# AnonymWriter/Iris-Style-Transfer

Measured on NVIDIA B200. Metric: masked-NST image-steps/sec @640x400 VGG-19, higher is better.
Workload: dtype bf16

## Files before the change

### include/isx.h

```cpp
#ifndef ISX_H_
#define ISX_H_

#include <stdint.h>

#ifdef __cplusplus
extern "C" {
#endif

#define ISX_VERSION 100

typedef uint16_t isx_bf16;
typedef void* isx_stream;

const char* isx_last_error(void);
int isx_version(void);
int isx_device_check(int device);

int isx_ipc_export(const void* ptr, void* handle64, int64_t* offset);
int isx_ipc_open(const void* handle64, void** base_out);
int isx_ipc_close(void* base);
int isx_copy_d2d_async(void* dst, const void* src, int64_t bytes, isx_stream stream);

typedef void* isx_handle;
int isx_create(int device, isx_handle* out);
// ... 20 lines not shown
                              int H, int W, int Cin, int Cout, int relu, int tile_cfg, isx_stream stream);

int isx_conv3x3_bias_relu_pool_fwd(const isx_bf16* in, const isx_bf16* w_fwd, const float* bias, isx_bf16* out,
                                   isx_bf16* pool_out, int B, int H, int W, int Cin, int Cout, int tile_cfg,
                                   isx_stream stream);
int isx_conv3x3_bias_relu_pool_idx_fwd(const isx_bf16* in, const isx_bf16* w_fwd, const float* bias, isx_bf16* out,
                                       isx_bf16* pool_out, uint8_t* pool_idx, int skip_out, int B, int H, int W, int Cin,
                                       int Cout, int tile_cfg, isx_stream stream);

int isx_conv3x3_dgrad(const isx_bf16* dy, const isx_bf16* w_dgrad, isx_bf16* dx, int B, int H, int W, int Cin,
                      int Cout, const isx_bf16* relu_act, const isx_bf16* add_grad, const float* aff_a,
                      const float* aff_b, int tile_cfg, isx_stream stream);

int isx_conv3x3_dgrad_gram(const isx_bf16* dy, const isx_bf16* w_dgrad, isx_bf16* dx, int B, int H, int W, int Cin,
                           int Cout, const isx_bf16* act_below, const isx_bf16* gram_D, isx_stream stream);

int isx_maxpool2x2_fwd(const isx_bf16* in, isx_bf16* out, int B, int H, int W, int C, isx_stream stream);
int isx_maxpool2x2_bwd(const isx_bf16* dy_pooled, const isx_bf16* act_prepool, isx_bf16* dx, int B, int H, int W,
                       int C, isx_stream stream);
int isx_maxpool2x2_fwd_idx(const isx_bf16* in, isx_bf16* out, uint8_t* idx, int B, int H, int W, int C, isx_stream stream);
int isx_maxpool2x2_bwd_idx(const isx_bf16* dy_pooled, const uint8_t* idx, isx_bf16* dx, int B, int H, int W, int C,
                           isx_stream stream);

int64_t isx_gram_workspace_bytes(int B, int HW, int C);
int isx_gram_fwd(const isx_bf16* feat, int B, int HW, int C, float inv_n, void* workspace, float* G_out,
                 const float* target, int target_b, double loss_scale, double* loss, float grad_scale,
                 isx_bf16* D_out, isx_stream stream);
int64_t isx_gram_mask_flags_bytes(int mask_b, int HW, int C);
int isx_gram_masked_fwd(const isx_bf16* feat, int B, int HW, int C, const float* m, int mask_b, void* flags_ws,
                        isx_bf16* fm2, float inv_n, void* workspace, float* G_out, const float* target, int target_b,
// ... 144 lines not shown
```

### iris-style-transfer_b200/csrc/api_ops.cu

```cuda
#include "../../include/isx.h"
#include "isx_common.cuh"
#include "isx_internal.h"
#include "isx_kernels.h"

using namespace isx;
typedef __nv_bfloat16 bf16;

static inline cudaStream_t S(isx_stream s) { return reinterpret_cast<cudaStream_t>(s); }
static inline const bf16* P(const isx_bf16* p) { return reinterpret_cast<const bf16*>(p); }
static inline bf16* P(isx_bf16* p) { return reinterpret_cast<bf16*>(p); }

static void decode_tile_cfg(int cfg, ConvArgs* a) {
  if (cfg > 0) {
    a->force_bn = cfg / 100;
    a->force_mt = (cfg % 100) / 10;
    a->force_stages = cfg % 10;
  }
}

extern "C" int isx_pack_conv3x3_weights(const float* w, int Cout, int Cin, isx_bf16* wf, isx_bf16* wd,
                                        isx_stream stream) {
  ISX_REQUIRE(w && (wf || wd) && Cout > 0 && Cin > 0, "isx_pack_conv3x3_weights: bad arguments");
  return pack_conv_weights(w, Cout, Cin, P(wf), P(wd), S(stream));
}
// ... 84 lines not shown
  a.in = P(dy); a.weight = P(w_dgrad); a.out = P(dx);
  a.B = B; a.H = H; a.W = W; a.Cin = Cout; a.Cout = Cin; a.ntaps = 9;
  a.mask_act = P(relu_act); a.add_buf = P(add_grad); a.aff_a = aff_a; a.aff_b = aff_b;
  decode_tile_cfg(tile_cfg, &a);
  return conv_tc(a, S(stream));
}

extern "C" int isx_conv3x3_dgrad_gram(const isx_bf16* dy, const isx_bf16* w_dgrad, isx_bf16* dx, int B, int H, int W,
                                      int Cin, int Cout, const isx_bf16* act_below, const isx_bf16* gram_D,
                                      isx_stream stream) {
  ISX_REQUIRE(dy && w_dgrad && dx && act_below && gram_D, "isx_conv3x3_dgrad_gram: null pointer");
  ConvArgs a;
  a.in = P(dy); a.weight = P(w_dgrad); a.out = P(dx);
  a.B = B; a.H = H; a.W = W; a.Cin = Cout; a.Cout = Cin; a.ntaps = 9;
  a.mask_act = P(act_below); a.gram_act = P(act_below); a.gram_D = P(gram_D);
  return conv_tc(a, S(stream));
}

extern "C" int isx_maxpool2x2_fwd(const isx_bf16* in, isx_bf16* out, int B, int H, int W, int C, isx_stream stream) {
  ISX_REQUIRE(in && out, "isx_maxpool2x2_fwd: null pointer");
  return maxpool_fwd(P(in), P(out), B, H, W, C, S(stream));
}

extern "C" int isx_maxpool2x2_bwd(const isx_bf16* dy, const isx_bf16* act, isx_bf16* dx, int B, int H, int W, int C,
                                  isx_stream stream) {
  ISX_REQUIRE(dy && act && dx, "isx_maxpool2x2_bwd: null pointer");
  return maxpool_bwd(P(dy), P(act), P(dx), B, H, W, C, S(stream));
}

extern "C" int isx_maxpool2x2_fwd_idx(const isx_bf16* in, isx_bf16* out, uint8_t* idx, int B, int H, int W, int C,
// ... 159 lines not shown
```

### iris-style-transfer_b200/csrc/conv_c64.cu

```cuda
#include <algorithm>

#include "isx_common.cuh"
#include "isx_internal.h"
#include "isx_kernels.h"

namespace isx {

static constexpr int kC64Threads = 64 + 256;
static constexpr int kHalo = 18 * 16 * 128;
static constexpr int kTile = 128 * 128;

struct C64Params {
  int B, H, W, Cout;
  int tiles_x, tiles_y;
  long total_items;
  int halo_slots;
  int relu, fuse_pool, use_mask, use_gram;
  const float* bias;
  const __nv_bfloat16* add_buf;
  const float* aff_a;
  const float* aff_b;
  float* dx_nchw;
  int xc;
  const float* in_mask;
// ... 387 lines not shown
      if (isx_make_tmap_bf16(&tmP, a.pool_out, 4, dp, sp, bp, true)) return 3;
    }
  }
  auto kern = conv_c64_kernel<BN, EPI>;
  ISX_CHECK_CUDA(cudaFuncSetAttribute(kern, cudaFuncAttributeMaxDynamicSharedMemorySize, (int)smem_bytes));
  const long grid = std::min<long>(p.total_items, kNumSMs);
  isx_prof_begin(ISX_PROF_CONV, 2.0 * (9 * 64 + (p.use_gram ? a.Cout : 0)) * a.Cout * static_cast<double>(a.B) * a.H * a.W, stream);
  kern<<<(unsigned)grid, kC64Threads, smem_bytes, stream>>>(tmA, tmW, tmO, tmM, tmD, tmP, p);
  isx_prof_end(ISX_PROF_CONV, stream);
  ISX_LAUNCH_CHECK();
  return 0;
}

bool conv_c64_applicable(const ConvArgs& a) {
  if (a.Cin != 64 || a.ntaps != 9 || a.per_image_weights) return false;
  if (a.dx_nchw != nullptr) return a.Cout == 16;
  if (a.Cout != 64) return false;
  if (a.gram_act != nullptr && a.gram_act != a.mask_act) return false;
  return true;
}

int conv_c64(const ConvArgs& a, cudaStream_t stream) {
  ISX_REQUIRE(conv_c64_applicable(a), "conv_c64: not applicable");
  if (a.dx_nchw != nullptr) return launch_c64<16, 1>(a, stream);
  return launch_c64<64, 0>(a, stream);
}

}
```

### iris-style-transfer_b200/csrc/conv_halo.cu

```cuda
#include <algorithm>

#include "isx_common.cuh"
#include "isx_internal.h"
#include "isx_kernels.h"

namespace isx {

static constexpr int kHaloThreads = 64 + 256;
static constexpr int kHaloSlot = 43 * 1024;
static constexpr int kSub = 128 * 128;

struct HaloParams {
  int B, H, W, Cin, Cout;
  int pairs_x, pairs_y, n_tiles;
  int total_items;
  int cin_blocks, extra_kb;
  int w_stages;
  int relu, fuse_pool, use_mask;
  const float* bias;
  const __nv_bfloat16* add_buf;
  const float* aff_a;
  const float* aff_b;
  uint8_t* pool_idx;
  int skip_out;
};

struct HaloLayout {
  int halo, w, act, stg, pstg, bars, total;
};
template <int BN>
__host__ __device__ inline HaloLayout halo_layout(int w_stages, int use_mask, int fuse_pool) {
  HaloLayout L;
  int off = 0;
  L.halo = off; off += 2 * kHaloSlot;
  L.w = off; off += w_stages * BN * 128;
  L.act = off; off += use_mask ? 2 * kSub : 0;
  L.stg = off; off += 2 * kSub;
  L.pstg = off; off += fuse_pool ? 2 * 4096 : 0;
  L.bars = off; off += 512;
  L.total = off;
  return L;
}

template <bool VERT>
struct ItemWalk {
  int b, r, stride, per_img, pairs_x, n_tiles;
  __device__ ItemWalk(int first, int stride_, int per_img_, int pairs_x_, int n_tiles_)
      : b(first / per_img_), r(first % per_img_), stride(stride_), per_img(per_img_), pairs_x(pairs_x_), n_tiles(n_tiles_) {}
  __device__ void next() {
    r += stride;
    while (r >= per_img) { r -= per_img; ++b; }
  }
  __device__ int nt() const { return r % n_tiles; }
// ... 6 lines not shown
conv_halo_kernel(const __grid_constant__ CUtensorMap tmA, const __grid_constant__ CUtensorMap tmW,
                 const __grid_constant__ CUtensorMap tmO, const __grid_constant__ CUtensorMap tmM,
                 const __grid_constant__ CUtensorMap tmA2, const __grid_constant__ CUtensorMap tmD,
                 const __grid_constant__ CUtensorMap tmP, const HaloParams p) {
  constexpr int kPitch = VERT ? 10 : 18;
  constexpr int kPatchRows = VERT ? 34 : 18;
  constexpr int kHaloBytes = kPitch * kPatchRows * 128;
  constexpr int kMtOff = VERT ? 16 * kPitch * 128 : 8 * 128;
  constexpr int kWStage = BN * 128;
  constexpr int kNH = BN / 64;
  constexpr int kNSub = 2 * kNH;
  constexpr int kAccCols = 2 * BN;
  constexpr int kTmemCols = 2 * kAccCols;
  extern __shared__ uint8_t smem_raw[];
  uint8_t* smem = reinterpret_cast<uint8_t*>((reinterpret_cast<uintptr_t>(smem_raw) + 1023) & ~uintptr_t(1023));
  const HaloLayout L = halo_layout<BN>(p.w_stages, p.use_mask, p.fuse_pool);
  const int WS = p.w_stages;
  uint64_t* bars = reinterpret_cast<uint64_t*>(smem + L.bars);
  uint64_t* halo_full = bars;
  uint64_t* halo_empty = bars + 2;
  uint64_t* w_full = bars + 4;
  uint64_t* w_empty = bars + 12;
  uint64_t* act_full = bars + 20;
  uint64_t* tmem_full = bars + 22;
  uint64_t* tmem_empty = bars + 24;
  uint32_t* tmem_ptr_smem = reinterpret_cast<uint32_t*>(bars + 26);

  const int warp = threadIdx.x >> 5;
  const int lane = threadIdx.x & 31;

  if (warp == 0 && lane == 0) {
// ... 138 lines not shown
    const int tw = row & 7, th = row >> 3;
    const bool leader = threadIdx.x == 64;
    ItemWalk<VERT> it(blockIdx.x, gridDim.x, per_img, p.pairs_x, p.n_tiles);
    auto issue_mask_load = [&](const ItemWalk<VERT>& w, int s, uint32_t g) {
      const int mt = s / kNH, nh = s - mt * kNH;
      const uint32_t slot = g & 1;
      mbar_arrive_expect_tx(&act_full[slot], kSub);
      tma_load_4d(smem + L.act + slot * kSub, &tmM, &act_full[slot], w.nt() * BN + nh * 64,
                  w.x0() + (VERT ? 0 : 8 * mt), w.y0() + (VERT ? 16 * mt : 0), w.b);
    };
    uint32_t g = 0;
    if (p.use_mask && leader && n_my > 0) {
      issue_mask_load(it, 0, 0);
      issue_mask_load(it, 1, 1);
    }
    uint32_t acc = 0, aph = 0;
    for (int i = 0; i < n_my; ++i) {
      const int b = it.b, x0 = it.x0(), y0 = it.y0(), n0 = it.nt() * BN;
      ItemWalk<VERT> nxt = it;
      nxt.next();
      mbar_wait(&tmem_full[acc], aph);
      tc_fence_after();
#pragma unroll 1
      for (int s = 0; s < kNSub; ++s, ++g) {
        const int mt = s / kNH, nh = s - mt * kNH;
        const int xs = x0 + (VERT ? 0 : 8 * mt), ys = y0 + (VERT ? 16 * mt : 0);
        const int nc = n0 + nh * 64 + hsel * 32;
        const int x = xs + tw, y = ys + th;
        const bool valid = (x < p.W) && (y < p.H);
        const size_t pix = valid ? ((static_cast<size_t>(b) * p.H + y) * p.W + x) * p.Cout : 0;
// ... 59 lines not shown
#pragma unroll
        for (int c = 0; c < 4; ++c) {
          uint4 o;
          o.x = pack_bf16x2(f[c * 8 + 0], f[c * 8 + 1]);
          o.y = pack_bf16x2(f[c * 8 + 2], f[c * 8 + 3]);
          o.z = pack_bf16x2(f[c * 8 + 4], f[c * 8 + 5]);
          o.w = pack_bf16x2(f[c * 8 + 6], f[c * 8 + 7]);
          const int chunk = (hsel * 4 + c) ^ (row & 7);
          *reinterpret_cast<uint4*>(rowp + chunk * 16) = o;
        }
        fence_proxy_async_smem();
        if (leader) tma_store_wait_read<0>();
        asm volatile("bar.sync 1, 256;" ::: "memory");
        const bool inside = xs < p.W && ys < p.H;
        if (leader) {
          if (inside && !p.skip_out) {
            tma_store_4d(&tmO, stg, n0 + nh * 64, xs, ys, b);
            tma_store_commit();
          }
          if (p.use_mask) {
            if (s + 2 < kNSub) issue_mask_load(it, s + 2, g + 2);
            else if (i + 1 < n_my) issue_mask_load(nxt, s + 2 - kNSub, g + 2);
          }
        }
        if (p.fuse_pool) {
          uint8_t* pst = smem + L.pstg + slot * 4096;
          const int item = threadIdx.x - 64;
          const int pr = item >> 3, chunk = item & 7;
          const int px = pr & 3, py = pr >> 2;
          const int r00 = (2 * py) * 8 + 2 * px;
          const int rr[4] = {r00, r00 + 1, r00 + 8, r00 + 9};
          uint4 u4[4];
#pragma unroll
          for (int k = 0; k < 4; ++k) u4[k] = *reinterpret_cast<const uint4*>(stg + rr[k] * 128 + ((chunk ^ (rr[k] & 7)) * 16));
          uint4 m4;
          uint2 codes;
          pool4_codes(u4, m4, codes);
          if (p.pool_idx != nullptr) {
// ... 32 lines not shown
  memset(&p, 0, sizeof(p));
  p.B = a.B; p.H = a.H; p.W = a.W; p.Cin = a.Cin; p.Cout = a.Cout;
  p.pairs_x = VERT ? (a.W + 7) / 8 : (a.W + 15) / 16;
  p.pairs_y = VERT ? (a.H + 31) / 32 : (a.H + 15) / 16;
  p.n_tiles = a.Cout / BN;
  const long total = static_cast<long>(p.pairs_x) * p.pairs_y * p.n_tiles * a.B;
  ISX_REQUIRE(total < (1L << 31) - kNumSMs, "conv_halo: too many work items");
  p.total_items = static_cast<int>(total);
  p.cin_blocks = a.Cin / 64;
  p.extra_kb = a.gram_act != nullptr ? a.Cout / 64 : 0;
  p.relu = a.relu; p.bias = a.bias; p.add_buf = a.add_buf; p.aff_a = a.aff_a; p.aff_b = a.aff_b;
  p.use_mask = a.mask_act != nullptr ? 1 : 0;
  p.fuse_pool = (a.pool_out != nullptr && a.H >= 2 && a.W >= 2) ? 1 : 0;
  p.pool_idx = p.fuse_pool ? a.pool_idx : nullptr;
  p.skip_out = (p.fuse_pool && a.pool_idx != nullptr && a.skip_out) ? 1 : 0;
  int ws = 6;
  HaloLayout L = halo_layout<BN>(ws, p.use_mask, p.fuse_pool);
  const int cap = (227 - std::max(0, std::min(isx_ctx()->opt_smem_reserve_kb, 22))) * 1024;
  while (ws > 2 && 1024 + L.total > cap) { --ws; L = halo_layout<BN>(ws, p.use_mask, p.fuse_pool); }
  ISX_REQUIRE(1024 + L.total <= 227 * 1024, "conv_halo: %d B of shared memory exceed 227 KB", 1024 + L.total);
  p.w_stages = ws;
  const size_t smem_bytes = std::max<size_t>(1024 + L.total, 204 * 1024);

  CUtensorMap tmA, tmW, tmO, tmM, tmA2, tmD, tmP;
  {
    uint64_t dims[4] = {(uint64_t)a.Cin, (uint64_t)a.W, (uint64_t)a.H, (uint64_t)a.B};
    uint64_t str[3] = {(uint64_t)a.Cin * 2, (uint64_t)a.W * a.Cin * 2, (uint64_t)a.H * a.W * a.Cin * 2};
    uint32_t box[4] = {64, VERT ? 10u : 18u, VERT ? 34u : 18u, 1};
    if (isx_make_tmap_bf16(&tmA, a.in, 4, dims, str, box, true)) return 3;
  }
  {
    uint64_t dims[2] = {(uint64_t)a.Cin, (uint64_t)9 * a.Cout};
    uint64_t str[1] = {(uint64_t)a.Cin * 2};
    uint32_t box[2] = {64, (uint32_t)BN};
// ... 63 lines not shown
```

### iris-style-transfer_b200/csrc/conv_sweep.cu

```cuda
#include <algorithm>

#include "isx_common.cuh"
#include "isx_internal.h"
#include "isx_kernels.h"

namespace isx {

static constexpr int kSwThreads = 64 + 256;
static constexpr int kSwPatch = 17 * 1024;
static constexpr int kSwPatchBytes = 130 * 128;
static constexpr int kSwTile = 128 * 128;
static constexpr int kSwWBytes = 9 * 64 * 128;
static constexpr int kSwMaxCtas = 160;

struct SweepParams {
  int B, H, W;
  int U, V;
  int u_is_y;
  int u_tiles;
  long total_cols;
  int cut_b[kSwMaxCtas + 1], cut_t[kSwMaxCtas + 1], cut_v[kSwMaxCtas + 1];
  int patch_slots;
  int relu, fuse_pool, use_mask, use_gram, skip_out;
  const float* bias;
// ... 529 lines not shown
    }
    tc_fence_before();
  }
  __syncthreads();
  if (warp == 1) {
    tc_fence_after();
    tmem_dealloc<512>(tmem_base);
  }
}

static double strip_efficiency(int n) { return static_cast<double>(n) / (((n + 127) / 128) * 128); }

bool conv_sweep_applicable(const ConvArgs& a) {
  if (a.Cin != 64 || a.Cout != 64 || a.ntaps != 9 || a.per_image_weights || a.dx_nchw != nullptr) return false;
  if (a.out == nullptr) return false;
  if (a.gram_act != nullptr && a.gram_act != a.mask_act) return false;
  if (a.aff_a != nullptr && a.mask_act == nullptr) return false;
  return true;
}
double conv_sweep_efficiency(const ConvArgs& a) { return std::max(strip_efficiency(a.H), strip_efficiency(a.W)); }

int conv_sweep(const ConvArgs& a, cudaStream_t stream) {
  ISX_REQUIRE(conv_sweep_applicable(a), "conv_sweep: not applicable");
  SweepParams p;
  memset(&p, 0, sizeof(p));
  p.B = a.B; p.H = a.H; p.W = a.W;
  p.u_is_y = strip_efficiency(a.H) > strip_efficiency(a.W) ? 1 : 0;
  p.U = p.u_is_y ? a.H : a.W;
  p.V = p.u_is_y ? a.W : a.H;
  p.u_tiles = (p.U + 127) / 128;
// ... 67 lines not shown
```

### iris-style-transfer_b200/csrc/conv_tc.cu

```cuda
#include "isx_common.cuh"
#include "isx_internal.h"
#include "isx_kernels.h"

namespace isx {

struct ConvParams {
  int B, H, W, Cin, Cout;
  int ntaps;
  int TW, TH, TB;
  int tiles_x, tiles_y, tiles_b;
  int n_tiles;
  int w_rows_per_image;
  int extra_kb;
  int stages;
  int relu;
  const float* bias;
  const __nv_bfloat16* mask_act;
  const __nv_bfloat16* add_buf;
  const float* aff_a;
  const float* aff_b;
  int fuse_pool;
  uint8_t* pool_idx;
  int skip_out;
  float* dx_nchw;
  int xc;
  const float* in_mask;
  int mask_b;
};

static constexpr int kATileBytes = 128 * 128;

static constexpr int kConvThreads = 64 + 256;

template <int BN, int MT, int EPI>
__global__ void __launch_bounds__(kConvThreads, 2)
conv_tc_kernel(const __grid_constant__ CUtensorMap tmA, const __grid_constant__ CUtensorMap tmB,
               const __grid_constant__ CUtensorMap tmO, const __grid_constant__ CUtensorMap tmM,
               const __grid_constant__ CUtensorMap tmA2, const __grid_constant__ CUtensorMap tmB2,
// ... 149 lines not shown
        }
      }
    } else {
    constexpr int NG = MT * (BN / 64);
    uint8_t* scratch = smem + NG * kATileBytes;
    const bool use_mask = p.mask_act != nullptr;
    auto issue_mask_load = [&](int gi) {
      const int mt_ = gi / (BN / 64), g_ = gi % (BN / 64);
      mbar_arrive_expect_tx(&epi_bar[gi & 1], kATileBytes);
      tma_load_4d(scratch + (gi & 1) * kATileBytes, &tmM, &epi_bar[gi & 1], n0 + g_ * 64, x0[mt_], y0[mt_], b0[mt_]);
    };
    if (use_mask && threadIdx.x == 64) {
      issue_mask_load(0);
      if (NG > 1) issue_mask_load(1);
    }
#pragma unroll 1
    for (int mt = 0; mt < MT; ++mt) {
      const int x = x0[mt] + tw, y = y0[mt] + th, b = b0[mt] + tb;
      const bool valid = (x < p.W) && (y < p.H) && (b < p.B);
      const size_t pix = valid ? ((static_cast<size_t>(b) * p.H + y) * p.W + x) * p.Cout : 0;
#pragma unroll 1
      for (int g = 0; g < BN / 64; ++g) {
        const int gi = mt * (BN / 64) + g;
        uint8_t* stg = smem + gi * kATileBytes;
        const uint8_t* mrow = scratch + (gi & 1) * kATileBytes + row * 128;
        if (use_mask) mbar_wait(&epi_bar[gi & 1], (gi >> 1) & 1);
        {
          const int h = hsel;
          const int nloc = g * 64 + h * 32;
          uint32_t v[32];
// ... 49 lines not shown
          uint8_t* rowp = stg + row * 128;
#pragma unroll
          for (int c = 0; c < 4; ++c) {
            uint4 o;
            o.x = pack_bf16x2(f[c * 8 + 0], f[c * 8 + 1]);
            o.y = pack_bf16x2(f[c * 8 + 2], f[c * 8 + 3]);
            o.z = pack_bf16x2(f[c * 8 + 4], f[c * 8 + 5]);
            o.w = pack_bf16x2(f[c * 8 + 6], f[c * 8 + 7]);
            const int chunk = (h * 4 + c) ^ (row & 7);
            *reinterpret_cast<uint4*>(rowp + chunk * 16) = o;
          }
        }
        fence_proxy_async_smem();
        asm volatile("bar.sync 1, 256;" ::: "memory");
        if (threadIdx.x == 64) {
          if (!p.skip_out) {
            tma_store_4d(&tmO, stg, n0 + g * 64, x0[mt], y0[mt], b0[mt]);
            tma_store_commit();
          }
          if (use_mask && gi + 2 < NG) issue_mask_load(gi + 2);
        }
        if (p.fuse_pool) {
          uint8_t* pst = smem + (NG + (use_mask ? 2 : 0)) * kATileBytes + gi * 4096;
          const int twp = p.TW >> 1, thp = p.TH >> 1;
          const int et = threadIdx.x - 64;
          {
            const int item = et;
            const int pr = item >> 3, chunk = item & 7;
            const int px = pr % twp, py = (pr / twp) % thp, pb = pr / (twp * thp);
            const int r00 = (pb * p.TH + 2 * py) * p.TW + 2 * px;
            const int rr[4] = {r00, r00 + 1, r00 + p.TW, r00 + p.TW + 1};
            uint4 u4[4];
#pragma unroll
            for (int k = 0; k < 4; ++k) u4[k] = *reinterpret_cast<const uint4*>(stg + rr[k] * 128 + ((chunk ^ (rr[k] & 7)) * 16));
            uint4 m4;
// ... 56 lines not shown
  p.n_tiles = a.Cout / BN;
  p.w_rows_per_image = a.per_image_weights ? a.Cout : 0;
  p.relu = a.relu; p.bias = a.bias; p.mask_act = a.mask_act; p.add_buf = a.add_buf;
  p.aff_a = a.aff_a; p.aff_b = a.aff_b;
  p.dx_nchw = a.dx_nchw; p.xc = a.xc; p.in_mask = a.in_mask; p.mask_b = a.mask_b;
  p.extra_kb = a.gram_act != nullptr ? a.Cout / 64 : 0;
  if (per_image && MT != 1)
    ISX_REQUIRE(p.TB == 1 && (p.tiles_x * p.tiles_y) % MT == 0, "per-image weights: an odd tile count per image needs MT = 1");

  constexpr int kStageBytes = MT * kATileBytes + BN * 128;
  const bool fuse_pool = EPI == 0 && a.pool_out != nullptr && p.TW % 2 == 0 && p.TH % 2 == 0 &&
                         a.H >= 2 && a.W >= 2;
  p.fuse_pool = fuse_pool ? 1 : 0;
  p.pool_idx = fuse_pool ? a.pool_idx : nullptr;
  p.skip_out = (fuse_pool && a.pool_idx != nullptr && a.skip_out) ? 1 : 0;
  const int epi_bytes = (MT * (BN / 64) + (a.mask_act ? 2 : 0)) * kATileBytes + (fuse_pool ? MT * (BN / 64) * 4096 : 0);
  int stages;
  size_t ring_bytes;
  stages = stages_override > 0 ? stages_override : (200 * 1024) / kStageBytes;
  if (stages > 8) stages = 8;
  if (stages < 2) stages = 2;
  while (stages * kStageBytes < epi_bytes) ++stages;
  ring_bytes = static_cast<size_t>(stages) * kStageBytes;
  p.stages = stages;
  const size_t smem_bytes = 1024 + ring_bytes + 256;
  ISX_REQUIRE(smem_bytes <= 227 * 1024, "conv_tc: %zu B of shared memory exceed 227 KB", smem_bytes);

  CUtensorMap tmA, tmB, tmO, tmM, tmA2, tmB2, tmP;
  {
    uint64_t dims[4] = {(uint64_t)a.Cin, (uint64_t)a.W, (uint64_t)a.H, (uint64_t)a.B};
    uint64_t str[3] = {(uint64_t)a.Cin * 2, (uint64_t)a.W * a.Cin * 2, (uint64_t)a.H * a.W * a.Cin * 2};
// ... 44 lines not shown
  ISX_CHECK_CUDA(cudaFuncSetAttribute(kern, cudaFuncAttributeMaxDynamicSharedMemorySize, (int)smem_bytes));
  isx_prof_begin(ISX_PROF_CONV,
                 2.0 * (a.ntaps * a.Cin + (a.gram_act ? a.Cout : 0)) * a.Cout * static_cast<double>(a.B) * a.H * a.W, stream);
  kern<<<(unsigned)grid, kConvThreads, smem_bytes, stream>>>(tmA, tmB, tmO, tmM, tmA2, tmB2, tmP, p);
  isx_prof_end(ISX_PROF_CONV, stream);
  ISX_LAUNCH_CHECK();
  if (a.pool_out != nullptr && !fuse_pool) {
    if (a.pool_idx != nullptr) return maxpool_fwd_idx(a.out, a.pool_out, a.pool_idx, a.B, a.H, a.W, a.Cout, stream);
    return maxpool_fwd(a.out, a.pool_out, a.B, a.H, a.W, a.Cout, stream);
  }
  return 0;
}

int conv_tc(const ConvArgs& a_in, cudaStream_t stream) {
  ConvArgs a = a_in;
  if (a.dx_nchw != nullptr && isx_ctx()->opt_tail_n > 0 && isx_ctx()->opt_c64 < 2 && a.force_bn == 0 &&
      a.Cin == 64 && a.Cout == 16 && a.ntaps == 9)
    return conv1_1_tail_n(a.in, a.weight, a.in_mask, a.mask_b, a.dx_nchw, a.xc, a.B, a.H, a.W, stream);
  if (isx_ctx()->opt_sweep64 > 0 && a.force_bn == 0 && conv_sweep_applicable(a)) {
    const long strips = static_cast<long>(a.B) * ((std::max(a.H, a.W) + 127) / 128) * std::min(a.H, a.W);
    if (isx_ctx()->opt_sweep64 >= 2 ||
        (conv_sweep_efficiency(a) >= 0.85 && strips >= 64L * kNumSMs && std::min(a.H, a.W) >= 16))
      return conv_sweep(a, stream);
  }
  if (isx_ctx()->opt_c64 > 0 && a.force_bn == 0 && conv_c64_applicable(a) &&
      (isx_ctx()->opt_c64 >= 2 || (a.dx_nchw == nullptr && static_cast<long>(a.B) * ((a.H + 15) / 16) * ((a.W + 7) / 8) >= kNumSMs)))
    return conv_c64(a, stream);
  if (isx_ctx()->opt_halo2 > 0 && a.force_bn == 0 && conv_halo_applicable(a)) {
    const long items = static_cast<long>(a.B) * ((a.H + 15) / 16) * ((a.W + 15) / 16) * (a.Cout / (a.Cout % 128 == 0 ? 128 : 64));
    if (isx_ctx()->opt_halo2 >= 2 || (items >= 2 * kNumSMs && conv_halo_efficiency(a) >= 0.85)) return conv_halo(a, stream);
// ... 40 lines not shown
```

### iris-style-transfer_b200/csrc/elementwise.cu

```cuda
#include <algorithm>

#include "isx_common.cuh"
#include "isx_internal.h"
#include "isx_kernels.h"

namespace isx {

__constant__ float c_mean[3] = {0.485f, 0.456f, 0.406f};
__constant__ float c_std[3] = {0.229f, 0.224f, 0.225f};

__global__ void pack_w_kernel(const float* __restrict__ w, int Cout, int Cin, __nv_bfloat16* __restrict__ wf,
                              __nv_bfloat16* __restrict__ wd) {
  const long n = static_cast<long>(Cout) * Cin * 9;
  for (long i = blockIdx.x * static_cast<long>(blockDim.x) + threadIdx.x; i < n;
       i += static_cast<long>(gridDim.x) * blockDim.x) {
    const int tap = i % 9;
    const int ci = (i / 9) % Cin;
    const int co = i / (9L * Cin);
    const __nv_bfloat16 v = __float2bfloat16_rn(w[i]);
    if (wf) wf[(static_cast<long>(tap) * Cout + co) * Cin + ci] = v;
    if (wd) wd[(static_cast<long>(8 - tap) * Cin + ci) * Cout + co] = v;
  }
}

// ... 271 lines not shown
}

__global__ void maxpool_bwd_idx_kernel(const __nv_bfloat16* __restrict__ dy, const uint8_t* __restrict__ idx,
                                       __nv_bfloat16* __restrict__ dx, int B, int H, int W, int C) {
  const int Ho = H / 2, Wo = W / 2, C8 = C / 8;
  const long n = static_cast<long>(B) * Ho * Wo * C8;
  for (long i = blockIdx.x * static_cast<long>(blockDim.x) + threadIdx.x; i < n;
       i += static_cast<long>(gridDim.x) * blockDim.x) {
    const int c8 = i % C8;
    const int xo = (i / C8) % Wo;
    const int yo = (i / (static_cast<long>(C8) * Wo)) % Ho;
    const int b = i / (static_cast<long>(C8) * Wo * Ho);
    const long po = ((static_cast<long>(b) * Ho + yo) * Wo + xo) * C + c8 * 8;
    const uint4 g = __ldg(reinterpret_cast<const uint4*>(dy + po));
    const uint2 cd = __ldg(reinterpret_cast<const uint2*>(idx + po));
    const uint32_t gw[4] = {g.x, g.y, g.z, g.w};
    const uint32_t c16[4] = {__byte_perm(cd.x, 0u, 0x4140), __byte_perm(cd.x, 0u, 0x4342), __byte_perm(cd.y, 0u, 0x4140),
                             __byte_perm(cd.y, 0u, 0x4342)};
    const long base = ((static_cast<long>(b) * H + 2 * yo) * W + 2 * xo) * C + c8 * 8;
    const long offs[4] = {0, C, static_cast<long>(W) * C, static_cast<long>(W) * C + C};
#pragma unroll
    for (int k = 0; k < 4; ++k) {
      uint32_t o[4];
#pragma unroll
      for (int e = 0; e < 4; ++e) {
        const uint32_t d = c16[e] ^ (static_cast<uint32_t>(k) * 0x00010001u);
        const uint32_t keep = ((d & 0x0000FFFFu) ? 0u : 0x0000FFFFu) | ((d & 0xFFFF0000u) ? 0u : 0xFFFF0000u);
        o[e] = gw[e] & keep;
      }
      *reinterpret_cast<uint4*>(dx + base + offs[k]) = make_uint4(o[0], o[1], o[2], o[3]);
    }
  }
}

int maxpool_bwd_idx(const __nv_bfloat16* dy, const uint8_t* idx, __nv_bfloat16* dx, int B, int H, int W, int C,
                    cudaStream_t s) {
  ISX_REQUIRE(C % 8 == 0 && H >= 2 && W >= 2, "maxpool_bwd: bad shape H=%d W=%d C=%d", H, W, C);
  if ((H & 1) || (W & 1))
    ISX_CHECK_CUDA(cudaMemsetAsync(dx, 0, static_cast<size_t>(B) * H * W * C * 2, s));
  const long n = static_cast<long>(B) * (H / 2) * (W / 2) * (C / 8);
  const int blocks = static_cast<int>(std::min<long>((n + 255) / 256, static_cast<long>(isx_num_sms()) * 16));
  maxpool_bwd_idx_kernel<<<blocks, 256, 0, s>>>(dy, idx, dx, B, H, W, C);
  ISX_LAUNCH_CHECK();
  return 0;
}

// ... 354 lines not shown
```

### iris-style-transfer_b200/csrc/isx_common.cuh

```cuda
#pragma once
#include <cuda.h>
#include <cuda_bf16.h>
#include <cuda_runtime.h>
#include <stdint.h>
#include <stdio.h>
#include <string.h>

void isx_set_error(const char* fmt, ...);

#define ISX_CHECK_CUDA(expr)                                                              \
  do {                                                                                    \
    cudaError_t _e = (expr);                                                              \
    if (_e != cudaSuccess) {                                                              \
      isx_set_error("%s:%d: %s -> %s", __FILE__, __LINE__, #expr, cudaGetErrorString(_e)); \
      return 1;                                                                           \
    }                                                                                     \
  } while (0)

#define ISX_REQUIRE(cond, ...)   \
  do {                           \
    if (!(cond)) {               \
      isx_set_error(__VA_ARGS__); \
      return 2;                  \
    }                            \
// ... 228 lines not shown
    uint32_t code = 0u;
#pragma unroll
    for (int k = 1; k < 4; ++k) {
      const __nv_bfloat162 a = reinterpret_cast<const __nv_bfloat162*>(&u[k])[e];
      const uint32_t gt = __hgt2_mask(a, m);
      m = __hmax2(m, a);
      code = (code & ~gt) | (gt & (static_cast<uint32_t>(k) * 0x00010001u));
    }
    const uint32_t z = __hle2_mask(m, zero2);
    cw[e] = (code & ~z) | (z & 0x00040004u);
    reinterpret_cast<__nv_bfloat162*>(&m4)[e] = m;
  }
  codes.x = __byte_perm(cw[0], cw[1], 0x6420);
  codes.y = __byte_perm(cw[2], cw[3], 0x6420);
}

__device__ __forceinline__ float warp_sum(float v) {
#pragma unroll
  for (int o = 16; o > 0; o >>= 1) v += __shfl_xor_sync(0xffffffffu, v, o);
  return v;
}
__device__ __forceinline__ double warp_sum(double v) {
#pragma unroll
  for (int o = 16; o > 0; o >>= 1) v += __shfl_xor_sync(0xffffffffu, v, o);
  return v;
}
__device__ __forceinline__ float warp_max(float v) {
#pragma unroll
  for (int o = 16; o > 0; o >>= 1) v = fmaxf(v, __shfl_xor_sync(0xffffffffu, v, o));
  return v;
// ... 5 lines not shown
```

### iris-style-transfer_b200/csrc/isx_internal.h

```cpp
#pragma once
#include <cuda_bf16.h>
#include <cuda_runtime.h>
#include <stdint.h>

namespace isx {

struct ConvArgs {
  const __nv_bfloat16* in = nullptr;
  const __nv_bfloat16* weight = nullptr;
  __nv_bfloat16* out = nullptr;
  int B = 0, H = 0, W = 0, Cin = 0, Cout = 0, ntaps = 9;
  bool per_image_weights = false;
  const float* bias = nullptr;
  int relu = 0;
  __nv_bfloat16* pool_out = nullptr;
  uint8_t* pool_idx = nullptr;
  bool skip_out = false;
  const __nv_bfloat16* mask_act = nullptr;
  const __nv_bfloat16* add_buf = nullptr;
  const float* aff_a = nullptr;
  const float* aff_b = nullptr;
  int force_bn = 0, force_mt = 0, force_stages = 0;
  const __nv_bfloat16* gram_act = nullptr;
  const __nv_bfloat16* gram_D = nullptr;
  float* dx_nchw = nullptr;
  int xc = 3;
  const float* in_mask = nullptr;
  int mask_b = 0;
};
int conv_tc(const ConvArgs& a, cudaStream_t stream);
bool conv_c64_applicable(const ConvArgs& a);
int conv_c64(const ConvArgs& a, cudaStream_t stream);
// ... 25 lines not shown
```

### iris-style-transfer_b200/csrc/nst_engine.cu

```cuda
#include <vector>

#include "../../include/isx.h"
#include "isx_common.cuh"
#include "isx_internal.h"
#include "isx_kernels.h"
#include "lbfgs_state.h"

using namespace isx;
typedef __nv_bfloat16 bf16;

static inline cudaStream_t S(isx_stream s) { return reinterpret_cast<cudaStream_t>(s); }

static const int kCout[16] = {64, 64, 128, 128, 256, 256, 256, 256, 512, 512, 512, 512, 512, 512, 512, 512};
static const int kCin[16] = {3, 64, 64, 128, 128, 256, 256, 256, 256, 512, 512, 512, 512, 512, 512, 512};
static const int kLevel[16] = {0, 0, 1, 1, 2, 2, 2, 2, 3, 3, 3, 3, 4, 4, 4, 4};
static inline bool pool_after(int i) { return i == 1 || i == 3 || i == 7 || i == 11 || i == 15; }
static const int kConvBefore[5] = {1, 3, 7, 11, 15};
static inline int pool_index(int conv) { return conv == 1 ? 0 : conv == 3 ? 1 : conv == 7 ? 2 : conv == 11 ? 3 : 4; }
static inline bool tap_is_pool(int id) { return id >= ISX_TAP_POOL0; }
static inline int tap_conv(int id) { return tap_is_pool(id) ? kConvBefore[id - ISX_TAP_POOL0] : id; }
static inline int tap_level(int id) { return tap_is_pool(id) ? id - ISX_TAP_POOL0 + 1 : kLevel[id]; }
static inline int tap_C(int id) { return kCout[tap_conv(id)]; }

namespace {
// ... 271 lines not shown
    const long HWj = static_cast<long>(L.H[lvj]) * L.W[lvj];
    const TapSrc& t = src[j];
    const bool through_pool = pool_after(j);
    ConvArgs a;
    a.in = gm; a.weight = reinterpret_cast<const bf16*>(b->w_dgrad[i]);
    ISX_REQUIRE(b->w_dgrad[i] != nullptr, "nst: packed dgrad weights of conv %d missing", i);
    a.B = B; a.H = L.H[lv]; a.W = L.W[lv]; a.Cin = kCout[i]; a.Cout = kCin[i]; a.ntaps = 9;
    a.out = (gm == ping) ? pong : ping;
    bf16* other = (a.out == ping) ? pong : ping;
    if (!through_pool) {
      a.mask_act = at(b, L.act[j]); a.add_buf = t.add; a.aff_a = t.aa; a.aff_b = t.ab;
      if (t.gram_D) { a.gram_act = t.gram_A; a.gram_D = t.gram_D; }
      if (int rc = conv_tc(a, s)) return rc;
      gm = a.out;
    } else {
      if (int rc = conv_tc(a, s)) return rc;
      if (pool_src(j))
        if (int rc = pool_combine(pool_index(j), a.out, a.out)) return rc;
      if (int rc = pool_bwd(a.out, lvj, j, other)) return rc;
      gm = other;
      if (t.any()) {
        const bf16* add2 = t.add;
        if (t.gram_D) {
          if (int rc = gram_1x1(j, tapbuf, false)) return rc;
          if (t.add) {
            if (int rc = tap_add_mask(t.add, tapbuf, nullptr, nullptr, at(b, L.act[j]), tapbuf, B, HWj, Cj, s)) return rc;
          }
          add2 = tapbuf;
        }
        if (int rc = tap_add_mask(other, add2, t.aa, t.ab, at(b, L.act[j]), a.out, B, HWj, Cj, s)) return rc;
        gm = a.out;
      }
    }
  }
// ... 251 lines not shown
```

Baseline: 2075.

## Fuse max-pool backward scatter into the dgrad conv epilogue

Adds an unpool epilogue to the tensor-core and halo dgrad conv kernels. It prefetches the pool argmax codes with cp.async and writes the gradient directly into the 2x-upsampled full-resolution buffer. This removes the separate maxpool-bwd launch and the round trip of the pre-pool gradient through global memory for pool layers whose pool output is not a style or content tap. The cost is extra shared memory, which can shrink the weight stages, and per-thread scattered stores in place of the TMA store.

```diff
diff --git a/include/isx.h b/include/isx.h
--- a/include/isx.h
+++ b/include/isx.h
@@ -58,6 +58,9 @@
 
 int isx_conv3x3_dgrad_gram(const isx_bf16* dy, const isx_bf16* w_dgrad, isx_bf16* dx, int B, int H, int W, int Cin,
                            int Cout, const isx_bf16* act_below, const isx_bf16* gram_D, isx_stream stream);
+
+int isx_conv3x3_dgrad_unpool(const isx_bf16* dy, const isx_bf16* w_dgrad, const uint8_t* pool_idx, isx_bf16* dx_full, int B,
+                             int H, int W, int Cin, int Cout, int tile_cfg, isx_stream stream);
 
 int isx_maxpool2x2_fwd(const isx_bf16* in, isx_bf16* out, int B, int H, int W, int C, isx_stream stream);
 int isx_maxpool2x2_bwd(const isx_bf16* dy_pooled, const isx_bf16* act_prepool, isx_bf16* dx, int B, int H, int W,
diff --git a/iris-style-transfer_b200/csrc/api_ops.cu b/iris-style-transfer_b200/csrc/api_ops.cu
--- a/iris-style-transfer_b200/csrc/api_ops.cu
+++ b/iris-style-transfer_b200/csrc/api_ops.cu
@@ -122,6 +122,16 @@
   a.in = P(dy); a.weight = P(w_dgrad); a.out = P(dx);
   a.B = B; a.H = H; a.W = W; a.Cin = Cout; a.Cout = Cin; a.ntaps = 9;
   a.mask_act = P(act_below); a.gram_act = P(act_below); a.gram_D = P(gram_D);
+  return conv_tc(a, S(stream));
+}
+
+extern "C" int isx_conv3x3_dgrad_unpool(const isx_bf16* dy, const isx_bf16* w_dgrad, const uint8_t* pool_idx, isx_bf16* dx_full,
+                                        int B, int H, int W, int Cin, int Cout, int tile_cfg, isx_stream stream) {
+  ISX_REQUIRE(dy && w_dgrad && pool_idx && dx_full, "isx_conv3x3_dgrad_unpool: null pointer");
+  ConvArgs a;
+  a.in = P(dy); a.weight = P(w_dgrad); a.out = P(dx_full); a.unpool_idx = pool_idx;
+  a.B = B; a.H = H; a.W = W; a.Cin = Cout; a.Cout = Cin; a.ntaps = 9;
+  decode_tile_cfg(tile_cfg, &a);
   return conv_tc(a, S(stream));
 }
 
diff --git a/iris-style-transfer_b200/csrc/conv_c64.cu b/iris-style-transfer_b200/csrc/conv_c64.cu
--- a/iris-style-transfer_b200/csrc/conv_c64.cu
+++ b/iris-style-transfer_b200/csrc/conv_c64.cu
@@ -425,6 +425,7 @@
 
 bool conv_c64_applicable(const ConvArgs& a) {
   if (a.Cin != 64 || a.ntaps != 9 || a.per_image_weights) return false;
+  if (a.unpool_idx != nullptr) return false;
   if (a.dx_nchw != nullptr) return a.Cout == 16;
   if (a.Cout != 64) return false;
   if (a.gram_act != nullptr && a.gram_act != a.mask_act) return false;
diff --git a/iris-style-transfer_b200/csrc/conv_halo.cu b/iris-style-transfer_b200/csrc/conv_halo.cu
--- a/iris-style-transfer_b200/csrc/conv_halo.cu
+++ b/iris-style-transfer_b200/csrc/conv_halo.cu
@@ -23,13 +23,15 @@
   const float* aff_b;
   uint8_t* pool_idx;
   int skip_out;
+  const uint8_t* unpool_idx;
+  __nv_bfloat16* unpool_out;
 };
 
 struct HaloLayout {
-  int halo, w, act, stg, pstg, bars, total;
+  int halo, w, act, stg, pstg, codes, bars, total;
 };
 template <int BN>
-__host__ __device__ inline HaloLayout halo_layout(int w_stages, int use_mask, int fuse_pool) {
+__host__ __device__ inline HaloLayout halo_layout(int w_stages, int use_mask, int fuse_pool, int unpool) {
   HaloLayout L;
   int off = 0;
   L.halo = off; off += 2 * kHaloSlot;
@@ -37,6 +39,7 @@
   L.act = off; off += use_mask ? 2 * kSub : 0;
   L.stg = off; off += 2 * kSub;
   L.pstg = off; off += fuse_pool ? 2 * 4096 : 0;
+  L.codes = off; off += unpool ? 8192 : 0;
   L.bars = off; off += 512;
   L.total = off;
   return L;
@@ -73,7 +76,7 @@
   constexpr int kTmemCols = 2 * kAccCols;
   extern __shared__ uint8_t smem_raw[];
   uint8_t* smem = reinterpret_cast<uint8_t*>((reinterpret_cast<uintptr_t>(smem_raw) + 1023) & ~uintptr_t(1023));
-  const HaloLayout L = halo_layout<BN>(p.w_stages, p.use_mask, p.fuse_pool);
+  const HaloLayout L = halo_layout<BN>(p.w_stages, p.use_mask, p.fuse_pool, p.unpool_out != nullptr);
   const int WS = p.w_stages;
   uint64_t* bars = reinterpret_cast<uint64_t*>(smem + L.bars);
   uint64_t* halo_full = bars;
@@ -242,6 +245,20 @@
       issue_mask_load(it, 0, 0);
       issue_mask_load(it, 1, 1);
     }
+    const int et = threadIdx.x - 64, uchunk = et & 7;
+    uint8_t* codes = smem + L.codes + et * 8;
+    auto fetch_codes = [&](const ItemWalk<VERT>& w, int s) {
+      const int mt = s / kNH, nh = s - mt * kNH;
+      const int xs = w.x0() + (VERT ? 0 : 8 * mt), ys = w.y0() + (VERT ? 16 * mt : 0);
+#pragma unroll
+      for (int k = 0; k < 4; ++k) {
+        const int pr = k * 32 + (et >> 3), x = xs + (pr & 7), y = ys + (pr >> 3);
+        if (x < p.W && y < p.H)
+          cp_async_8(codes + k * 2048, p.unpool_idx + ((static_cast<size_t>(w.b) * p.H + y) * p.W + x) * p.Cout + w.nt() * BN +
+                                           nh * 64 + uchunk * 8);
+      }
+    };
+    if (p.unpool_out != nullptr && n_my > 0) fetch_codes(it, 0);
     uint32_t acc = 0, aph = 0;
     for (int i = 0; i < n_my; ++i) {
       const int b = it.b, x0 = it.x0(), y0 = it.y0(), n0 = it.nt() * BN;
@@ -331,7 +348,7 @@
         asm volatile("bar.sync 1, 256;" ::: "memory");
         const bool inside = xs < p.W && ys < p.H;
         if (leader) {
-          if (inside && !p.skip_out) {
+          if (inside && !p.skip_out && p.unpool_out == nullptr) {
             tma_store_4d(&tmO, stg, n0 + nh * 64, xs, ys, b);
             tma_store_commit();
           }
@@ -339,6 +356,22 @@
             if (s + 2 < kNSub) issue_mask_load(it, s + 2, g + 2);
             else if (i + 1 < n_my) issue_mask_load(nxt, s + 2 - kNSub, g + 2);
           }
+        }
+        if (p.unpool_out != nullptr) {
+          const long Wf = 2L * p.W;
+          cp_async_wait_all();
+#pragma unroll
+          for (int k = 0; k < 4; ++k) {
+            const int pr = k * 32 + (et >> 3), x = xs + (pr & 7), y = ys + (pr >> 3);
+            if (x < p.W && y < p.H) {
+              const uint4 v = *reinterpret_cast<const uint4*>(stg + pr * 128 + ((uchunk ^ (pr & 7)) * 16));
+              const uint2 cd = *reinterpret_cast<const uint2*>(codes + k * 2048);
+              unpool4_store(v, cd, p.unpool_out + ((static_cast<long>(b) * 2 * p.H + 2 * y) * Wf + 2 * x) * p.Cout + n0 + nh * 64 + uchunk * 8,
+                            p.Cout, Wf * p.Cout);
+            }
+          }
+          if (s + 1 < kNSub) fetch_codes(it, s + 1);
+          else if (i + 1 < n_my) fetch_codes(nxt, 0);
         }
         if (p.fuse_pool) {
           uint8_t* pst = smem + L.pstg + slot * 4096;
@@ -401,10 +434,13 @@
   p.fuse_pool = (a.pool_out != nullptr && a.H >= 2 && a.W >= 2) ? 1 : 0;
   p.pool_idx = p.fuse_pool ? a.pool_idx : nullptr;
   p.skip_out = (p.fuse_pool && a.pool_idx != nullptr && a.skip_out) ? 1 : 0;
+  p.unpool_idx = a.unpool_idx;
+  p.unpool_out = a.unpool_idx != nullptr ? a.out : nullptr;
   int ws = 6;
-  HaloLayout L = halo_layout<BN>(ws, p.use_mask, p.fuse_pool);
+  const int unpool = p.unpool_out != nullptr;
+  HaloLayout L = halo_layout<BN>(ws, p.use_mask, p.fuse_pool, unpool);
   const int cap = (227 - std::max(0, std::min(isx_ctx()->opt_smem_reserve_kb, 22))) * 1024;
-  while (ws > 2 && 1024 + L.total > cap) { --ws; L = halo_layout<BN>(ws, p.use_mask, p.fuse_pool); }
+  while (ws > 2 && 1024 + L.total > cap) { --ws; L = halo_layout<BN>(ws, p.use_mask, p.fuse_pool, unpool); }
   ISX_REQUIRE(1024 + L.total <= 227 * 1024, "conv_halo: %d B of shared memory exceed 227 KB", 1024 + L.total);
   p.w_stages = ws;
   const size_t smem_bytes = std::max<size_t>(1024 + L.total, 204 * 1024);
diff --git a/iris-style-transfer_b200/csrc/conv_sweep.cu b/iris-style-transfer_b200/csrc/conv_sweep.cu
--- a/iris-style-transfer_b200/csrc/conv_sweep.cu
+++ b/iris-style-transfer_b200/csrc/conv_sweep.cu
@@ -567,6 +567,7 @@
 bool conv_sweep_applicable(const ConvArgs& a) {
   if (a.Cin != 64 || a.Cout != 64 || a.ntaps != 9 || a.per_image_weights || a.dx_nchw != nullptr) return false;
   if (a.out == nullptr) return false;
+  if (a.unpool_idx != nullptr) return false;
   if (a.gram_act != nullptr && a.gram_act != a.mask_act) return false;
   if (a.aff_a != nullptr && a.mask_act == nullptr) return false;
   return true;
diff --git a/iris-style-transfer_b200/csrc/conv_tc.cu b/iris-style-transfer_b200/csrc/conv_tc.cu
--- a/iris-style-transfer_b200/csrc/conv_tc.cu
+++ b/iris-style-transfer_b200/csrc/conv_tc.cu
@@ -22,6 +22,8 @@
   int fuse_pool;
   uint8_t* pool_idx;
   int skip_out;
+  const uint8_t* unpool_idx;
+  __nv_bfloat16* unpool_out;
   float* dx_nchw;
   int xc;
   const float* in_mask;
@@ -201,6 +203,24 @@
       issue_mask_load(0);
       if (NG > 1) issue_mask_load(1);
     }
+    const int et = threadIdx.x - 64, uchunk = et & 7;
+    uint8_t* codes = scratch + (use_mask ? 2 : 0) * kATileBytes + et * 8;
+    auto unpool_pixel = [&](int mt, int k, int& ux, int& uy, int& ub) -> bool {
+      const int r = k * 32 + (et >> 3);
+      const int m = mt == 0 ? 0 : MT - 1;
+      ux = x0[m] + r % p.TW; uy = y0[m] + (r / p.TW) % p.TH; ub = b0[m] + r / (p.TW * p.TH);
+      return ux < p.W && uy < p.H && ub < p.B;
+    };
+    auto fetch_codes = [&](int gi) {
+      const int mt = gi / (BN / 64), g = gi % (BN / 64);
+#pragma unroll
+      for (int k = 0; k < 4; ++k) {
+        int ux, uy, ub;
+        if (unpool_pixel(mt, k, ux, uy, ub))
+          cp_async_8(codes + k * 2048, p.unpool_idx + ((static_cast<size_t>(ub) * p.H + uy) * p.W + ux) * p.Cout + n0 + g * 64 + uchunk * 8);
+      }
+    };
+    if (p.unpool_out != nullptr) fetch_codes(0);
 #pragma unroll 1
     for (int mt = 0; mt < MT; ++mt) {
       const int x = x0[mt] + tw, y = y0[mt] + th, b = b0[mt] + tb;
@@ -280,11 +300,27 @@
         fence_proxy_async_smem();
         asm volatile("bar.sync 1, 256;" ::: "memory");
         if (threadIdx.x == 64) {
-          if (!p.skip_out) {
+          if (!p.skip_out && p.unpool_out == nullptr) {
             tma_store_4d(&tmO, stg, n0 + g * 64, x0[mt], y0[mt], b0[mt]);
             tma_store_commit();
           }
           if (use_mask && gi + 2 < NG) issue_mask_load(gi + 2);
+        }
+        if (p.unpool_out != nullptr) {
+          const long Wf = 2L * p.W;
+          cp_async_wait_all();
+#pragma unroll
+          for (int k = 0; k < 4; ++k) {
+            int ux, uy, ub;
+            if (unpool_pixel(mt, k, ux, uy, ub)) {
+              const int r = k * 32 + (et >> 3);
+              const uint4 v = *reinterpret_cast<const uint4*>(stg + r * 128 + ((uchunk ^ (r & 7)) * 16));
+              const uint2 cd = *reinterpret_cast<const uint2*>(codes + k * 2048);
+              unpool4_store(v, cd, p.unpool_out + ((static_cast<long>(ub) * 2 * p.H + 2 * uy) * Wf + 2 * ux) * p.Cout + n0 + g * 64 + uchunk * 8,
+                            p.Cout, Wf * p.Cout);
+            }
+          }
+          if (gi + 1 < NG) fetch_codes(gi + 1);
         }
         if (p.fuse_pool) {
           uint8_t* pst = smem + (NG + (use_mask ? 2 : 0)) * kATileBytes + gi * 4096;
@@ -371,7 +407,10 @@
   p.fuse_pool = fuse_pool ? 1 : 0;
   p.pool_idx = fuse_pool ? a.pool_idx : nullptr;
   p.skip_out = (fuse_pool && a.pool_idx != nullptr && a.skip_out) ? 1 : 0;
-  const int epi_bytes = (MT * (BN / 64) + (a.mask_act ? 2 : 0)) * kATileBytes + (fuse_pool ? MT * (BN / 64) * 4096 : 0);
+  p.unpool_idx = a.unpool_idx;
+  p.unpool_out = a.unpool_idx != nullptr ? a.out : nullptr;
+  const int epi_bytes = (MT * (BN / 64) + (a.mask_act ? 2 : 0)) * kATileBytes + (fuse_pool ? MT * (BN / 64) * 4096 : 0) +
+                        (a.unpool_idx ? 8192 : 0);
   int stages;
   size_t ring_bytes;
   stages = stages_override > 0 ? stages_override : (200 * 1024) / kStageBytes;
@@ -446,6 +485,10 @@
 
 int conv_tc(const ConvArgs& a_in, cudaStream_t stream) {
   ConvArgs a = a_in;
+  ISX_REQUIRE(a.unpool_idx == nullptr ||
+                  (a.ntaps == 9 && a.out != nullptr && !a.per_image_weights && a.bias == nullptr && !a.relu && a.pool_out == nullptr &&
+                   a.mask_act == nullptr && a.add_buf == nullptr && a.aff_a == nullptr && a.gram_act == nullptr && a.dx_nchw == nullptr),
+              "conv: the max-pool backward epilogue (unpool_idx) takes a plain 3x3 dgrad");
   if (a.dx_nchw != nullptr && isx_ctx()->opt_tail_n > 0 && isx_ctx()->opt_c64 < 2 && a.force_bn == 0 &&
       a.Cin == 64 && a.Cout == 16 && a.ntaps == 9)
     return conv1_1_tail_n(a.in, a.weight, a.in_mask, a.mask_b, a.dx_nchw, a.xc, a.B, a.H, a.W, stream);
diff --git a/iris-style-transfer_b200/csrc/elementwise.cu b/iris-style-transfer_b200/csrc/elementwise.cu
--- a/iris-style-transfer_b200/csrc/elementwise.cu
+++ b/iris-style-transfer_b200/csrc/elementwise.cu
@@ -309,22 +309,8 @@
     const long po = ((static_cast<long>(b) * Ho + yo) * Wo + xo) * C + c8 * 8;
     const uint4 g = __ldg(reinterpret_cast<const uint4*>(dy + po));
     const uint2 cd = __ldg(reinterpret_cast<const uint2*>(idx + po));
-    const uint32_t gw[4] = {g.x, g.y, g.z, g.w};
-    const uint32_t c16[4] = {__byte_perm(cd.x, 0u, 0x4140), __byte_perm(cd.x, 0u, 0x4342), __byte_perm(cd.y, 0u, 0x4140),
-                             __byte_perm(cd.y, 0u, 0x4342)};
     const long base = ((static_cast<long>(b) * H + 2 * yo) * W + 2 * xo) * C + c8 * 8;
-    const long offs[4] = {0, C, static_cast<long>(W) * C, static_cast<long>(W) * C + C};
-#pragma unroll
-    for (int k = 0; k < 4; ++k) {
-      uint32_t o[4];
-#pragma unroll
-      for (int e = 0; e < 4; ++e) {
-        const uint32_t d = c16[e] ^ (static_cast<uint32_t>(k) * 0x00010001u);
-        const uint32_t keep = ((d & 0x0000FFFFu) ? 0u : 0x0000FFFFu) | ((d & 0xFFFF0000u) ? 0u : 0xFFFF0000u);
-        o[e] = gw[e] & keep;
-      }
-      *reinterpret_cast<uint4*>(dx + base + offs[k]) = make_uint4(o[0], o[1], o[2], o[3]);
-    }
+    unpool4_store(g, cd, dx + base, C, static_cast<long>(W) * C);
   }
 }
 
diff --git a/iris-style-transfer_b200/csrc/isx_common.cuh b/iris-style-transfer_b200/csrc/isx_common.cuh
--- a/iris-style-transfer_b200/csrc/isx_common.cuh
+++ b/iris-style-transfer_b200/csrc/isx_common.cuh
@@ -266,6 +266,27 @@
   codes.x = __byte_perm(cw[0], cw[1], 0x6420);
   codes.y = __byte_perm(cw[2], cw[3], 0x6420);
 }
+__device__ __forceinline__ void cp_async_8(void* smem_dst, const void* gsrc) {
+  asm volatile("cp.async.ca.shared.global [%0], [%1], 8;" ::"r"(smem_u32(smem_dst)), "l"(gsrc) : "memory");
+}
+__device__ __forceinline__ void cp_async_wait_all() { asm volatile("cp.async.wait_all;" ::: "memory"); }
+__device__ __forceinline__ void unpool4_store(const uint4 g, const uint2 cd, __nv_bfloat16* dx, long c_stride, long row_stride) {
+  const uint32_t gw[4] = {g.x, g.y, g.z, g.w};
+  const uint32_t c16[4] = {__byte_perm(cd.x, 0u, 0x4140), __byte_perm(cd.x, 0u, 0x4342), __byte_perm(cd.y, 0u, 0x4140),
+                           __byte_perm(cd.y, 0u, 0x4342)};
+  const long offs[4] = {0, c_stride, row_stride, row_stride + c_stride};
+#pragma unroll
+  for (int k = 0; k < 4; ++k) {
+    uint32_t o[4];
+#pragma unroll
+    for (int e = 0; e < 4; ++e) {
+      const uint32_t d = c16[e] ^ (static_cast<uint32_t>(k) * 0x00010001u);
+      const uint32_t keep = ((d & 0x0000FFFFu) ? 0u : 0x0000FFFFu) | ((d & 0xFFFF0000u) ? 0u : 0xFFFF0000u);
+      o[e] = gw[e] & keep;
+    }
+    *reinterpret_cast<uint4*>(dx + offs[k]) = make_uint4(o[0], o[1], o[2], o[3]);
+  }
+}
 
 __device__ __forceinline__ float warp_sum(float v) {
 #pragma unroll
diff --git a/iris-style-transfer_b200/csrc/isx_internal.h b/iris-style-transfer_b200/csrc/isx_internal.h
--- a/iris-style-transfer_b200/csrc/isx_internal.h
+++ b/iris-style-transfer_b200/csrc/isx_internal.h
@@ -16,6 +16,7 @@
   __nv_bfloat16* pool_out = nullptr;
   uint8_t* pool_idx = nullptr;
   bool skip_out = false;
+  const uint8_t* unpool_idx = nullptr;
   const __nv_bfloat16* mask_act = nullptr;
   const __nv_bfloat16* add_buf = nullptr;
   const float* aff_a = nullptr;
diff --git a/iris-style-transfer_b200/csrc/nst_engine.cu b/iris-style-transfer_b200/csrc/nst_engine.cu
--- a/iris-style-transfer_b200/csrc/nst_engine.cu
+++ b/iris-style-transfer_b200/csrc/nst_engine.cu
@@ -1,3 +1,4 @@
+#include <utility>
 #include <vector>
 
 #include "../../include/isx.h"
@@ -309,10 +310,17 @@
       if (int rc = conv_tc(a, s)) return rc;
       gm = a.out;
     } else {
-      if (int rc = conv_tc(a, s)) return rc;
-      if (pool_src(j))
-        if (int rc = pool_combine(pool_index(j), a.out, a.out)) return rc;
-      if (int rc = pool_bwd(a.out, lvj, j, other)) return rc;
+      const bool fused = !pool_src(j) && (L.H[lvj] & 1) == 0 && (L.W[lvj] & 1) == 0;
+      if (fused) {
+        a.unpool_idx = atb(b, L.pidx[lvj]);
+        if (int rc = conv_tc(a, s)) return rc;
+        std::swap(a.out, other);
+      } else {
+        if (int rc = conv_tc(a, s)) return rc;
+        if (pool_src(j))
+          if (int rc = pool_combine(pool_index(j), a.out, a.out)) return rc;
+        if (int rc = pool_bwd(a.out, lvj, j, other)) return rc;
+      }
       gm = other;
       if (t.any()) {
         const bf16* add2 = t.add;
diff --git a/scratch/unpool_launches.py b/scratch/unpool_launches.py
--- /dev/null
+++ b/scratch/unpool_launches.py
@@ -0,0 +1,42 @@
+import sys
+from collections import defaultdict
+
+import torch
+
+sys.path.insert(0, ".")
+import bench
+import iris_b200
+from iris_b200 import pipelines
+
+out = sys.argv[1]
+dev = torch.device("cuda:0")
+B = 64
+vgg = iris_b200.VGG19(weights="random", seed=0)
+c, s = bench.make_inputs(B, 1, bench.H, bench.W)
+with torch.cuda.device(dev), torch.no_grad():
+    job = pipelines.NstJob(c.to(dev), s.to(dev), vgg, dev, clone_content=True, BN_loss=False, c_loss_weight=1.0,
+                           s_loss_weight=1e6, lr=1.0, epochs=200, independent=True, history_size=100)
+    for _ in range(110):
+        job.tick()
+    torch.cuda.synchronize()
+    with torch.profiler.profile(activities=[torch.profiler.ProfilerActivity.CUDA]) as prof:
+        job.tick()
+        torch.cuda.synchronize()
+kernels = [e for e in prof.events() if e.device_type == torch.autograd.DeviceType.CUDA]
+kernels.sort(key=lambda e: e.time_range.start)
+total = defaultdict(float)
+count = defaultdict(int)
+name = torch.cuda.get_device_name(0)
+with open(out, "w") as f:
+    f.write("# one nst640 tick (B = %d), %s; torch.profiler CUDA activities; us per launch and per image\n" % (B, name))
+    for e in kernels:
+        us = e.time_range.elapsed_us()
+        short = e.name.split("(")[0][:90]
+        total[short] += us
+        count[short] += 1
+        f.write("%10.1f us %8.2f us/img  %s\n" % (us, us / B, short))
+    f.write("\n# totals by kernel\n")
+    for k in sorted(total, key=lambda k: -total[k]):
+        f.write("%10.1f us %8.2f us/img %4d x  %s\n" % (total[k], total[k] / B, count[k], k))
+    f.write("# all kernels: %.1f us (%.2f us/img)\n" % (sum(total.values()), sum(total.values()) / B))
+print(open(out).read()[-3000:])
```

Measured after the change: 2090, median of 6. Within noise of the previous version (+0.8%).
